# Haian-Jin/TensoIR

Hardware: AMD Instinct MI355X
Metric: primary+secondary rays/sec at 4096 rays x 512 samples (higher is better)
Workload: dtype f32 io and field; decoders split-bf16 x3 (hi/lo operands, 3 MFMA products), fp32 accumulate; indirect light (secondary-ray records): fp16 shadow taps + fp16 single-product decoder, fp32 accumulate

## Files before the change

### include/tensoir_hip.h

```cpp
#ifndef TENSOIR_HIP_H
#define TENSOIR_HIP_H

#include <stdint.h>

#ifdef __cplusplus
extern "C" {
#endif

#define TIR_VERSION 100

#define TIR_OK               0
#define TIR_ERR_ARG         -1001
#define TIR_ERR_UNSUPPORTED -1002
#define TIR_ERR_NO_DEVICE   -1003

typedef struct TirField {
    float aabb_min[3];
    float aabb_max[3];
    float inv_aabb[3];
    int32_t grid[3];
    float step_size;
    float distance_scale;
    float density_shift;
    float weight_thres;
// ... 66 lines not shown
int tir_vm_density_fwd(const TirField* f, const float* xyz, float* feat, float* sigma,
                       int64_t n, void* stream);

int tir_occupancy_query(const TirField* f, const float* xyz, uint8_t* hit, int64_t n, void* stream);

int tir_dense_alpha(const TirField* f, const float* lin_x, const float* lin_y, const float* lin_z,
                    int32_t gx, int32_t gy, int32_t gz, float length, float* alpha, void* stream);
int tir_alpha_pool(const float* alpha, int32_t gx, int32_t gy, int32_t gz, float thres, float* vol,
                   int32_t* bbox, void* stream);
int tir_filter_rays(const TirField* f, const float* rays, int64_t n, int32_t n_samples, int32_t bbox_only,
                    uint8_t* mask, void* stream);

int tir_dense_sigma_build(const TirField* f, float* vol, int32_t pitch, void* stream);
int tir_dense_sigma_fwd(const TirField* f, const float* xyz, float* feat, float* sigma, int64_t n, void* stream);

int tir_dense_app_build(const TirField* f, void* vol, int32_t pitch, void* stream);

int tir_density_grad_fwd(const TirField* f, const float* xyz, float* sigma, float* grad,
                         float* normal, int64_t n, const int32_t* n_dev, void* stream);
int tir_density_feat_grad_fwd(const TirField* f, const float* xyz, float* feat, float* grad, int64_t n, void* stream);

int tir_vm_app_fwd(const TirField* f, const float* xyz, const int32_t* light_idx,
                   const int32_t* idx_map, float* rad_feat, float* int_feat, int32_t out_stride,
                   int32_t idx_div, int64_t n, const int32_t* n_dev, void* stream);

int tir_vm_app_jitter_fwd(const TirField* f, const float* xyz, int64_t n, const int32_t* n_dev, float scale,
                          uint64_t seed, uint64_t offset, const int64_t* rng_state, float* xyz_out,
                          float* int_feat, int32_t out_stride, void* stream);

int tir_vm_app_primary_fwd(const TirField* f, const float* xyz, const int32_t* light_idx, const int32_t* idx_map,
                           float* rad_feat, float* int_feat, int32_t out_stride, int64_t n, const int32_t* n_dev,
                           float scale, uint64_t seed, uint64_t offset, const int64_t* rng_state, float* xyz_out,
                           float* int_feat_jit, void* stream);
int tir_vm_app_primary_x3_fwd(const TirField* f, const float* xyz, const int32_t* light_idx, const int32_t* idx_map,
                              float* rad_feat, float* int_feat, int32_t out_stride, int64_t n, const int32_t* n_dev,
                              float scale, uint64_t seed, uint64_t offset, const int64_t* rng_state, float* xyz_out,
                              float* int_feat_jit, void* stream);
int tir_vm_app_fwd_x3(const TirField* f, const float* xyz, const int32_t* light_idx,
                      const int32_t* idx_map, float* rad_feat, float* int_feat, int32_t out_stride,
                      int32_t idx_div, int64_t n, const int32_t* n_dev, void* stream);
int tir_vm_app_fwd_bf16x3(const TirField* f, const float* xyz, const int32_t* light_idx,
                          const int32_t* idx_map, float* rad_feat, float* int_feat, int32_t out_stride,
                          int32_t idx_div, int64_t n, const int32_t* n_dev, void* stream);
int tir_vm_app_fwd_valu(const TirField* f, const float* xyz, const int32_t* light_idx,
                        const int32_t* idx_map, float* rad_feat, float* int_feat, int32_t out_stride,
                        int32_t idx_div, int64_t n, const int32_t* n_dev, void* stream);

int tir_mlp_fwd(const TirMlp* m, const float* feat, int32_t feat_stride, const float* aux,
                const int32_t* aux_map, int32_t aux_mod, float* out, int64_t n, const int32_t* n_dev,
        void* stream);
int tir_mlp_fwd_bf16x3(const TirMlp* m, const float* feat, int32_t feat_stride, const float* aux,
                       const int32_t* aux_map, int32_t aux_mod, float* out, int64_t n, const int32_t* n_dev,
        void* stream);

int tir_pack_half(const float* const* srcs, void* const* dsts, const int64_t* counts, int32_t n_tables, void* stream);
int tir_pack_half_checked(const float* const* srcs, void* const* dsts, const int64_t* counts, int32_t n_tables, float* absmax,
                          void* stream);
int tir_vm_app_fwd_h16(const TirField* f, const TirFieldHalf* fh, const float* xyz, const int32_t* light_idx,
                       const int32_t* idx_map, float* rad_feat, int32_t out_stride, int32_t idx_div, int64_t n,
                       const int32_t* n_dev, void* stream);

int tir_indirect_fused_fwd(const TirField* f, const TirFieldHalf* fh, const TirMlp* m, const float* xyz,
                           const int32_t* light_idx, const int32_t* rec_map, int32_t idx_div, int32_t aux_mod,
                           const float* table, float* out, int64_t n, const int32_t* n_dev, void* stream);

int tir_indirect_fused_hp_fwd(const TirField* f, const TirMlp* m, const float* xyz, const int32_t* light_idx,
// ... 434 lines not shown
```

### tensoir_amd/csrc/tir_common.hpp

```cpp
#pragma once
#include <hip/hip_runtime.h>
#include <stdint.h>
#include <initializer_list>
#include <type_traits>
#include "tensoir_hip.h"

#define TIR_WAVE 64

#define TIR_CHECK_LAUNCH()                                   \
    do {                                                     \
        hipError_t e__ = hipGetLastError();                  \
        if (e__ != hipSuccess) return -(int)e__;             \
    } while (0)

static inline hipStream_t tir_stream(void* s) { return reinterpret_cast<hipStream_t>(s); }

static inline int tir_xcd_mapping(const TirField* f) { return f->tune_xcd_order == 1 ? 1 : 0; }

#include <mutex>
#include <set>
#include <utility>
static inline int tir_allow_dynamic_lds(const void* kernel, int bytes) {
    static std::mutex mu;
    static std::set<std::pair<const void*, int>> done;
// ... 65 lines not shown
    int n_acomp = 0;
    int app_dim = 0;
    bool feature_rows = true;
    int stride_max = 32;
    TirAppNeeds& fp16_tables(const TirFieldHalf* fh) { half = fh; return *this; }
    TirAppNeeds& aligned() { aligned16 = true; return *this; }
    TirAppNeeds& no_light_mean() { light_mean = false; return *this; }
    TirAppNeeds& element_index32() { index32 = true; return *this; }
    TirAppNeeds& width(int n) { n_acomp = n; return *this; }
    TirAppNeeds& app_dim_is(int d) { app_dim = d; return *this; }
    TirAppNeeds& no_feature_rows() { feature_rows = false; return *this; }
    TirAppNeeds& stride_unbounded() { stride_max = 0x7fffffff; return *this; }
};

static inline int tir_check_app_field(const TirField* f, const TirAppNeeds& need, int out_stride) {
    for (int i = 0; i < 3; ++i) {
        const void* plane = need.half ? need.half->aplane[i] : static_cast<const void*>(f->aplane[i]);
        const void* line = need.half ? need.half->aline[i] : static_cast<const void*>(f->aline[i]);
        if (f->grid[i] < 2 || !plane || !line || (need.aligned16 && !tir_aligned16({plane, line}))) return TIR_ERR_ARG;
    }
    if (!f->basis_t || !f->light_line || (need.light_mean && !f->light_mean)) return TIR_ERR_ARG;
    if (need.n_acomp && f->n_acomp != need.n_acomp) return TIR_ERR_UNSUPPORTED;
    if (need.app_dim ? f->app_dim != need.app_dim : (f->app_dim < 1 || f->app_dim > 27)) return TIR_ERR_UNSUPPORTED;
    if (need.index32 && !tir_app_index_ok(f)) return TIR_ERR_UNSUPPORTED;
    if (need.feature_rows && (out_stride < f->app_dim || out_stride > need.stride_max)) return TIR_ERR_ARG;
    return TIR_OK;
}

template <typename Go>
static inline int tir_with_rows(int64_t n, std::initializer_list<const void*> need, std::initializer_list<const void*> aligned, Go&& go) {
    if (n < 0 || (n > 0 && tir_any_null(need)) || !tir_aligned16(aligned)) return TIR_ERR_ARG;
    if (n == 0) return TIR_OK;
    return go();
}

constexpr int TIR_APP_LDS_LIMIT = 160 * 1024;

static inline unsigned tir_gather_blocks(int64_t n, int rows, int cap, int xcd_on) {
    int64_t blocks = (n + rows - 1) / rows;
    if (blocks > cap) blocks = cap;
    if (xcd_on) blocks = (blocks + 7) / 8 * 8;
    return (unsigned)blocks;
}

static inline unsigned tir_job_split(int64_t units, int total, int n_jobs) {
    int per = total / n_jobs;
    if (per < 1) per = 1;
    if (units < per) per = (int)units;
    return (unsigned)(per * n_jobs);
}

template <typename... P, typename... A>
static inline int tir_launch(void (*kernel)(P...), int lds_limit, dim3 grid, dim3 block, size_t lds, hipStream_t s, const A&... args) {
    if (lds_limit > 0)
        if (int rc = tir_allow_dynamic_lds(reinterpret_cast<const void*>(kernel), lds_limit)) return rc;
    hipLaunchKernelGGL(kernel, grid, block, lds, s, args...);
    TIR_CHECK_LAUNCH();
    return TIR_OK;
}

template <int... C4S, typename Fn>
static inline int tir_dispatch_c4(int n_acomp, Fn&& fn) {
    int rc = TIR_ERR_UNSUPPORTED;
    (void)((n_acomp == 4 * C4S && ((rc = fn(std::integral_constant<int, C4S>{})), true)) || ...);
    return rc;
}
// ... 810 lines not shown
```

### tensoir_amd/csrc/tir_field.hip

```cpp
#include "tir_common.hpp"

using namespace tir;

__global__ void k_pack_plane(const float* __restrict__ src, float* __restrict__ dst, int C, int HW) {
    int64_t i = (int64_t)blockIdx.x * blockDim.x + threadIdx.x;
    if (i >= (int64_t)C * HW) return;
    int c = (int)(i % C);
    int64_t t = i / C;
    dst[i] = src[(int64_t)c * HW + t];
}

__global__ void k_pack_occ(const float* __restrict__ vol, uint8_t* __restrict__ nbr, int W, int H, int D) {
    int64_t i = (int64_t)blockIdx.x * blockDim.x + threadIdx.x;
    const int64_t n = (int64_t)(W + 1) * (H + 1) * (D + 1);
    if (i >= n) return;
    const int x0 = (int)(i % (W + 1)) - 1, y0 = (int)((i / (W + 1)) % (H + 1)) - 1, z0 = (int)(i / ((int64_t)(W + 1) * (H + 1))) - 1;
    uint32_t m = 0;
    for (int c = 0; c < 8; ++c) {
        const int xx = x0 + (c & 1), yy = y0 + ((c >> 1) & 1), zz = z0 + (c >> 2);
        if (xx >= 0 && xx < W && yy >= 0 && yy < H && zz >= 0 && zz < D && vol[((int64_t)zz * H + yy) * W + xx] > 0.5f) m |= 1u << c;
    }
    nbr[i] = (uint8_t)m;
}

// ... 234 lines not shown

extern "C" int tir_dense_sigma_fwd(const TirField* f, const float* xyz, float* feat, float* sigma, int64_t n, void* stream) {
    int rc = check_field(f);
    if (rc) return rc;
    if (n < 0 || (n > 0 && !xyz)) return TIR_ERR_ARG;
    if (!tir_dense_sigma_ok(f)) return TIR_ERR_UNSUPPORTED;
    if (n == 0) return TIR_OK;
    hipLaunchKernelGGL(k_dense_sigma_fwd, dim3((unsigned)((n + 255) / 256)), dim3(256), 0, tir_stream(stream), *f, xyz, feat, sigma, n);
    TIR_CHECK_LAUNCH();
    return TIR_OK;
}

extern "C" int tir_alpha_pool(const float* alpha, int32_t gx, int32_t gy, int32_t gz, float thres, float* vol,
                              int32_t* bbox, void* stream) {
    if (!alpha || !vol || gx <= 0 || gy <= 0 || gz <= 0) return TIR_ERR_ARG;
    const int64_t n = (int64_t)gx * gy * gz;
    hipLaunchKernelGGL(k_alpha_pool, dim3((unsigned)((n + 255) / 256)), dim3(256), 0, tir_stream(stream), alpha, gx, gy,
                       gz, thres, vol, bbox);
    TIR_CHECK_LAUNCH();
    return TIR_OK;
}

extern "C" int tir_filter_rays(const TirField* f, const float* rays, int64_t n, int32_t n_samples, int32_t bbox_only,
                               uint8_t* mask, void* stream) {
    if (!f || n < 0 || (n > 0 && (!rays || !mask))) return TIR_ERR_ARG;
    if (!bbox_only && (!f->occ_nbr || n_samples <= 0)) return TIR_ERR_ARG;
    if (n == 0) return TIR_OK;
    hipLaunchKernelGGL(k_filter_rays, dim3((unsigned)((n + 3) / 4)), dim3(256), 0, tir_stream(stream), *f, rays, n,
                       n_samples, bbox_only, mask);
    TIR_CHECK_LAUNCH();
    return TIR_OK;
}

template <int C4>
__device__ __forceinline__ void plane_line_grad(const float* __restrict__ plane, const float* __restrict__ line,
                                                int H, int W, int R, float u, float v, float w,
                                                float& val, float& du, float& dv, float& dw) {
    Tap1 tx = make_tap(u, W), ty = make_tap(v, H), tl = make_tap(w, R);
    const float wx0 = 1.0f - tx.t, wx1 = tx.t, wy0 = 1.0f - ty.t, wy1 = ty.t;
    const float* p00 = plane + ((size_t)ty.i0 * W + tx.i0) * (C4 * 4);
    const float* p01 = plane + ((size_t)ty.i0 * W + tx.i1) * (C4 * 4);
    const float* p10 = plane + ((size_t)ty.i1 * W + tx.i0) * (C4 * 4);
    const float* p11 = plane + ((size_t)ty.i1 * W + tx.i1) * (C4 * 4);
    const float* l0 = line + (size_t)tl.i0 * (C4 * 4);
    const float* l1 = line + (size_t)tl.i1 * (C4 * 4);
    const float sx = 0.5f * (float)(W - 1), sy = 0.5f * (float)(H - 1), sl = 0.5f * (float)(R - 1);
    float a_val = 0.f, a_du = 0.f, a_dv = 0.f, a_dw = 0.f;
#pragma unroll
    for (int c = 0; c < C4 * 4; ++c) {
        float a = p00[c], b = p01[c], cc = p10[c], d = p11[c], e = l0[c], g = l1[c];
        float P = fmaf(d, wx1 * wy1, fmaf(cc, wx0 * wy1, fmaf(b, wx1 * wy0, a * (wx0 * wy0))));
        float Pu = fmaf(d - cc, wy1, (b - a) * wy0);
        float Pv = fmaf(d - b, wx1, (cc - a) * wx0);
        float L = fmaf(g, tl.t, e * (1.0f - tl.t));
        float Lw = g - e;
        a_val = fmaf(P, L, a_val);
        a_du = fmaf(Pu, L, a_du);
        a_dv = fmaf(Pv, L, a_dv);
        a_dw = fmaf(P, Lw, a_dw);
    }
    val = a_val; du = a_du * sx; dv = a_dv * sy; dw = a_dw * sl;
}

template <int C4>
__global__ void __launch_bounds__(256)
k_density_grad(TirField f, const float* __restrict__ xyz, float* __restrict__ sigma,
               float* __restrict__ grad, float* __restrict__ normal, int64_t n, const int32_t* __restrict__ n_dev) {
    int64_t i = (int64_t)blockIdx.x * blockDim.x + threadIdx.x;
    if (n_dev) n = min(n, (int64_t)max(*n_dev, 0));
    if (i >= n) return;
    const float px = xyz[3 * i], py = xyz[3 * i + 1], pz = xyz[3 * i + 2];
    float g0 = 0.f, g1 = 0.f, g2 = 0.f;
    float feat = 0.f;
#pragma unroll 1
    for (int k = 0; k < 3; ++k) {
        const float u = (k == 2) ? py : px, v = (k == 0) ? py : pz, w = (k == 0) ? pz : ((k == 1) ? py : px);
        const int m0 = (k == 2) ? 1 : 0, m1 = (k == 0) ? 1 : 2, vi = 2 - k;
        float val, du, dv, dw;
        plane_line_grad<C4>(f.dplane[k], f.dline[k], f.grid[m1], f.grid[m0], f.grid[vi], u, v, w, val, du, dv, dw);
        feat += val;
        if (k == 0) { g0 += du; g1 += dv; g2 += dw; }
        else if (k == 1) { g0 += du; g2 += dv; g1 += dw; }
        else { g1 += du; g2 += dv; g0 += dw; }
    }
    const float g[3] = {g0, g1, g2};
    float ds, sg;
    if (f.act == 1) { sg = fmaxf(feat, 0.f); ds = feat > 0.f ? 1.f : 0.f; }
    else {
        float x = feat + f.density_shift;
        sg = softplus20(x);
        ds = (x > 20.f) ? 1.f : 1.0f / (1.0f + expf(-x));
    }
    float gx = ds * g[0], gy = ds * g[1], gz = ds * g[2];
    if (sigma) sigma[i] = sg;
    if (grad) { grad[3 * i] = gx; grad[3 * i + 1] = gy; grad[3 * i + 2] = gz; }
    if (normal) {
        float nrm = fmaxf(sqrtf(gx * gx + gy * gy + gz * gz), 1e-6f);
        normal[3 * i] = -gx / nrm; normal[3 * i + 1] = -gy / nrm; normal[3 * i + 2] = -gz / nrm;
    }
}

extern "C" int tir_density_grad_fwd(const TirField* f, const float* xyz, float* sigma, float* grad,
                                    float* normal, int64_t n, const int32_t* n_dev, void* stream) {
    int rc = check_field(f);
    if (rc) return rc;
    if (n < 0 || (n > 0 && !xyz)) return TIR_ERR_ARG;
    if (n == 0) return TIR_OK;
    dim3 g((unsigned)((n + 255) / 256)), b(256);
    switch (f->n_dcomp) {
        case 16: hipLaunchKernelGGL(k_density_grad<4>, g, b, 0, tir_stream(stream), *f, xyz, sigma, grad, normal, n, n_dev); break;
        case 8:  hipLaunchKernelGGL(k_density_grad<2>, g, b, 0, tir_stream(stream), *f, xyz, sigma, grad, normal, n, n_dev); break;
        case 32: hipLaunchKernelGGL(k_density_grad<8>, g, b, 0, tir_stream(stream), *f, xyz, sigma, grad, normal, n, n_dev); break;
        default: hipLaunchKernelGGL(k_density_grad<1>, g, b, 0, tir_stream(stream), *f, xyz, sigma, grad, normal, n, n_dev); break;
    }
    TIR_CHECK_LAUNCH();
    return TIR_OK;
}

template <int C4>
__global__ void __launch_bounds__(256)
k_density_feat_grad(TirField f, const float* __restrict__ xyz, float* __restrict__ feat, float* __restrict__ grad, int64_t n) {
    int64_t i = (int64_t)blockIdx.x * blockDim.x + threadIdx.x;
    if (i >= n) return;
    const float p[3] = {xyz[3 * i], xyz[3 * i + 1], xyz[3 * i + 2]};
    float g[3] = {0.f, 0.f, 0.f}, acc = 0.f;
#pragma unroll 1
    for (int k = 0; k < 3; ++k) {
        const int m0 = (k == 2) ? 1 : 0, m1 = (k == 0) ? 1 : 2, vi = 2 - k;
        float val, du, dv, dw;
        plane_line_grad<C4>(f.dplane[k], f.dline[k], f.grid[m1], f.grid[m0], f.grid[vi], p[m0], p[m1], p[vi], val, du, dv, dw);
        acc += val;
        g[m0] += du; g[m1] += dv; g[vi] += dw;
// ... 331 lines not shown
}

template <int C4, bool HX = false>
__global__ void __launch_bounds__(256)
k_vm_app_primary(TirField f, const float* __restrict__ xyz, const int32_t* __restrict__ light_idx,
                 const int32_t* __restrict__ idx_map, float* __restrict__ rad_feat, float* __restrict__ int_feat,
                 float* __restrict__ int_feat_jit, int out_stride, int64_t n, const int32_t* __restrict__ n_dev, int xcd_on,
                 TirJitter jt, int lt_rows, int nb0) {
    if ((int)blockIdx.x < nb0) {
        TirJitter none{0.0f, 0ull, 0ull, nullptr, nullptr};
        app_mfma_body<C4, true, true, false, HX>(f, xyz, light_idx, idx_map, rad_feat, int_feat, out_stride, 0, n, n_dev, xcd_on, none,
                                                 lt_rows, (int)blockIdx.x, nb0);
    } else {
        app_mfma_body<C4, false, true, true, HX>(f, xyz, nullptr, nullptr, nullptr, int_feat_jit, out_stride, 0, n, n_dev, xcd_on, jt,
                                                 lt_rows, (int)blockIdx.x - nb0, (int)gridDim.x - nb0);
    }
}

template <int C4, bool HX = false>
__global__ void __launch_bounds__(256)
k_vm_app_primary_one(TirField f, const float* __restrict__ xyz, float* __restrict__ rad_feat, float* __restrict__ int_feat,
                     float* __restrict__ int_feat_jit, int out_stride, int64_t n, const int32_t* __restrict__ n_dev, int xcd_on,
                     TirJitter jt, int nb0) {
    if ((int)blockIdx.x < nb0) {
        TirJitter none{0.0f, 0ull, 0ull, nullptr, nullptr};
        app_mfma_body<C4, true, true, false, HX, true>(f, xyz, nullptr, nullptr, rad_feat, int_feat, out_stride, 0, n, n_dev, xcd_on, none,
                                                       1, (int)blockIdx.x, nb0);
    } else {
        app_mfma_body<C4, false, true, true, HX>(f, xyz, nullptr, nullptr, nullptr, int_feat_jit, out_stride, 0, n, n_dev, xcd_on, jt,
                                                 0, (int)blockIdx.x - nb0, (int)gridDim.x - nb0);
    }
}

typedef __bf16 app_bf16x8 __attribute__((ext_vector_type(8)));
#define TIR_XS 68

__device__ __forceinline__ void app_split8(const float4& v0, const float4& v1, app_bf16x8& hi, app_bf16x8& lo) {
    const float v[8] = {v0.x, v0.y, v0.z, v0.w, v1.x, v1.y, v1.z, v1.w};
#pragma unroll
    for (int e = 0; e < 8; ++e) {
        hi[e] = (__bf16)v[e];
        lo[e] = (__bf16)(v[e] - (float)hi[e]);
    }
}

template <int C4, bool RAD, bool INTR>
__global__ void __launch_bounds__(256)
k_vm_app_bf16(TirField f, const float* __restrict__ xyz, const int32_t* __restrict__ light_idx,
              const int32_t* __restrict__ idx_map, float* __restrict__ rad_feat, float* __restrict__ int_feat,
              int out_stride, int idx_div, int64_t n, const int32_t* __restrict__ n_dev, int xcd_on) {
    static_assert(C4 * 4 <= 64, "one VM group must fit two 32-wide k-steps");
    if (n_dev) n = min(n, (int64_t)max(*n_dev, 0));
    constexpr int CA = C4 * 4;
    constexpr int NX = (RAD ? 1 : 0) + (INTR ? 1 : 0);
    extern __shared__ __attribute__((aligned(16))) float lds_app[];
    app_bf16x8* Whi = reinterpret_cast<app_bf16x8*>(lds_app);
    app_bf16x8* Wlo = Whi + 3 * 2 * 2 * 64;
    const int wave = threadIdx.x >> 6, L = threadIdx.x & 63;
    float* X = reinterpret_cast<float*>(Wlo + 3 * 2 * 2 * 64) + wave * (NX * 16 * TIR_XS);
    for (int e = threadIdx.x; e < 3 * 2 * 2 * 64; e += 256) {
        const int row = e & 15, kg = (e >> 4) & 3, mt = (e >> 6) & 1, t = (e >> 7) & 1, k = e >> 8;
        app_bf16x8 hi, lo;
#pragma unroll
        for (int q = 0; q < 8; ++q) {
            const int ch = 32 * t + 8 * kg + q;
            const float w = (ch < CA) ? f.basis_t[(size_t)(k * CA + ch) * 32 + mt * 16 + row] : 0.0f;
// ... 320 lines not shown
static int app_fwd(const TirField* f, const float* xyz, const int32_t* li, const int32_t* map, float* rad, float* intr,
                   int32_t stride, int32_t idx_div, int64_t n, const int32_t* n_dev, void* stream, AppContraction how,
                   const TirJitter& jt = TirJitter{0.0f, 0ull, 0ull, nullptr, nullptr}) {
    if (!f) return TIR_ERR_ARG;
    if (int rc = tir_check_app_field(f, TirAppNeeds(), stride)) return rc;
    if ((!rad && !intr) || (rad && !li)) return TIR_ERR_ARG;
    return tir_with_rows(n, {xyz}, {}, [&] {
        hipStream_t s = tir_stream(stream);
        if (how == APP_BF16X3) return tir_dispatch_c4<12, 6, 4>(f->n_acomp, [&](auto c4) { return launch_app_bf16<decltype(c4)::value>(f, xyz, li, map, rad, intr, stride, idx_div, n, n_dev, s); });
        if (how == APP_HX) return tir_dispatch_c4<12, 6, 4>(f->n_acomp, [&](auto c4) { return launch_app_hx<decltype(c4)::value>(f, xyz, li, map, rad, intr, stride, idx_div, n, n_dev, s); });
        return tir_dispatch_c4<12, 6, 4, 24>(f->n_acomp, [&](auto c4) { return launch_app<decltype(c4)::value>(f, xyz, li, map, rad, intr, stride, idx_div, n, n_dev, s, how == APP_VALU, jt); });
    });
}
#undef TIR_APP_ARGS

extern "C" int tir_vm_app_fwd(const TirField* f, const float* xyz, const int32_t* light_idx,
                              const int32_t* idx_map, float* rad_feat, float* int_feat, int32_t out_stride,
                              int32_t idx_div, int64_t n, const int32_t* n_dev, void* stream) {
    return app_fwd(f, xyz, light_idx, idx_map, rad_feat, int_feat, out_stride, idx_div, n, n_dev, stream, APP_FP32);
}

extern "C" int tir_vm_app_jitter_fwd(const TirField* f, const float* xyz, int64_t n, const int32_t* n_dev, float scale,
                                     uint64_t seed, uint64_t offset, const int64_t* rng_dev, float* xyz_out,
                                     float* int_feat, int32_t out_stride, void* stream) {
    if (!xyz_out || !int_feat || scale == 0.0f) return TIR_ERR_ARG;
    TirJitter jt{scale, (unsigned long long)seed, (unsigned long long)offset, reinterpret_cast<const long long*>(rng_dev), xyz_out};
    return app_fwd(f, xyz, nullptr, nullptr, nullptr, int_feat, out_stride, 0, n, n_dev, stream, APP_FP32, jt);
}

template <bool HX>
static int app_primary_fwd(const TirField* f, const float* xyz, const int32_t* light_idx, const int32_t* idx_map, float* rad_feat,
                           float* int_feat, int32_t out_stride, int64_t n, const int32_t* n_dev, float scale, uint64_t seed,
                           uint64_t offset, const int64_t* rng_state, float* xyz_out, float* int_feat_jit, void* stream) {
    if (!f || !rad_feat || !int_feat || !xyz_out || !int_feat_jit || !light_idx || scale == 0.0f) return TIR_ERR_ARG;
    if (int rc = tir_check_app_field(f, TirAppNeeds().width(48), out_stride)) return rc;
    return tir_with_rows(n, {xyz}, {}, [&] {
        constexpr int C4 = 12, CA = 48;
        const int lt_rows = f->n_lights <= 16 ? f->n_lights : 0;
        const size_t w_floats = HX ? (2 * 3 * 2 * 2 * 64 * 16) / 4 : 3 * CA * 32;
        const size_t x_floats = HX ? (2 * 2 * 16 * TIR_XHX * 2) / 4 : 2 * CA * TIR_XLD;
        const int nb = (int)tir_gather_blocks(n, 64, 1024, 1);
        const dim3 g(2 * nb), b(256);
        const int xcd_on = tir_xcd_mapping(f);
        const TirJitter jt{scale, (unsigned long long)seed, (unsigned long long)offset, reinterpret_cast<const long long*>(rng_state), xyz_out};
        if (f->n_lights == 1) {
            const size_t lds1 = (w_floats + (size_t)2 * 3 * CA + 4 * (x_floats / 2)) * sizeof(float);
            return tir_launch(k_vm_app_primary_one<C4, HX>, TIR_APP_LDS_LIMIT, g, b, lds1, tir_stream(stream), *f, xyz, rad_feat, int_feat,
                              int_feat_jit, out_stride, n, n_dev, xcd_on, jt, nb);
        }
        const size_t lds = (w_floats + (size_t)(lt_rows + 1) * 3 * CA + 4 * x_floats) * sizeof(float);
        return tir_launch(k_vm_app_primary<C4, HX>, TIR_APP_LDS_LIMIT, g, b, lds, tir_stream(stream), *f, xyz, light_idx, idx_map, rad_feat,
                          int_feat, int_feat_jit, out_stride, n, n_dev, xcd_on, jt, lt_rows, nb);
    });
}

extern "C" int tir_vm_app_primary_fwd(const TirField* f, const float* xyz, const int32_t* light_idx, const int32_t* idx_map,
                                      float* rad_feat, float* int_feat, int32_t out_stride, int64_t n, const int32_t* n_dev,
                                      float scale, uint64_t seed, uint64_t offset, const int64_t* rng_state, float* xyz_out,
                                      float* int_feat_jit, void* stream) {
    return app_primary_fwd<false>(f, xyz, light_idx, idx_map, rad_feat, int_feat, out_stride, n, n_dev, scale, seed, offset, rng_state,
                                  xyz_out, int_feat_jit, stream);
}

extern "C" int tir_vm_app_primary_x3_fwd(const TirField* f, const float* xyz, const int32_t* light_idx, const int32_t* idx_map,
                                         float* rad_feat, float* int_feat, int32_t out_stride, int64_t n, const int32_t* n_dev,
                                         float scale, uint64_t seed, uint64_t offset, const int64_t* rng_state, float* xyz_out,
                                         float* int_feat_jit, void* stream) {
    return app_primary_fwd<true>(f, xyz, light_idx, idx_map, rad_feat, int_feat, out_stride, n, n_dev, scale, seed, offset, rng_state,
                                 xyz_out, int_feat_jit, stream);
}

extern "C" int tir_vm_app_fwd_x3(const TirField* f, const float* xyz, const int32_t* light_idx,
                                 const int32_t* idx_map, float* rad_feat, float* int_feat, int32_t out_stride,
                                 int32_t idx_div, int64_t n, const int32_t* n_dev, void* stream) {
    return app_fwd(f, xyz, light_idx, idx_map, rad_feat, int_feat, out_stride, idx_div, n, n_dev, stream, APP_HX);
}

extern "C" int tir_vm_app_fwd_valu(const TirField* f, const float* xyz, const int32_t* light_idx,
                                   const int32_t* idx_map, float* rad_feat, float* int_feat, int32_t out_stride,
                                   int32_t idx_div, int64_t n, const int32_t* n_dev, void* stream) {
    return app_fwd(f, xyz, light_idx, idx_map, rad_feat, int_feat, out_stride, idx_div, n, n_dev, stream, APP_VALU);
}

extern "C" int tir_vm_app_fwd_bf16x3(const TirField* f, const float* xyz, const int32_t* light_idx,
                                     const int32_t* idx_map, float* rad_feat, float* int_feat, int32_t out_stride,
// ... 74 lines not shown
```

### tensoir_amd/field_model.py

```python
from __future__ import annotations

import functools
import math
import time

import numpy as np
import torch
import torch.nn as nn
import torch.nn.functional as F

from . import capacity, indirect, ops, regularisers
from ._lib import TensoirHipError, TirField

MAT_MODE = [[0, 1], [0, 2], [1, 2]]
VEC_MODE = [2, 1, 0]


def raw2alpha(sigma, dist):
    alpha = 1.0 - torch.exp(-sigma * dist)
    T = torch.cumprod(torch.cat([torch.ones(alpha.shape[0], 1).to(alpha.device), 1.0 - alpha + 1e-10], -1), -1)
    weights = alpha * T[:, :-1]
    return alpha, weights, T[:, -1:]


# ... 849 lines not shown
        f = self.packed_field()
        lidx = ops.to_device(light_idx.reshape(-1), dev, torch.int32).contiguous()
        jitter = ops.to_device(torch.rand(B, 1), dev) if is_train else None
        from . import training
        if training.wants_grad(self):
            bg = bool(white_bg or (is_train and torch.rand((1,)) < 0.5))
            for attempt in range(2):
                try:
                    maps = training.PrimaryRenderFn.apply(self, rays, lidx, S, bg, bool(is_relight), jitter,
                                                          _brdf_jitter_dense, bool(_defer_check),
                                                          *training.field_param_list(self))
                    break
                except training._CapacityOverflow:
                    if attempt:
                        raise
            out = self.unpack_maps(maps, is_relight, want_mask=_want_mask)
            return (out, maps) if _return_maps else out
        rc = capacity.PassCapacity(self.__dict__.setdefault("_app_cap_hints", {}), (B, S), 1.25, ceiling=B * S, max_entries=64,
                                   capture=self.__dict__.get("_capture"), check_key=("primary", B, S))
        cap = rc.hinted() if (not is_train and _brdf_jitter_dense is None) else None
        words = viewdirs = None
        if cap is None:
            weight, acc, depth, _tend, cnt = ops.march_primary(f, rays, jitter, S, self.march_t_stop)
            offsets = ops.exclusive_scan(cnt)
            A, n_dev = int(offsets[-1].item()), None
        else:
            words = self._step_words(dev)
            weight, acc, depth, cnt, offsets, total_dev, viewdirs = ops.march_primary_fused(f, rays, S, self.march_t_stop,
                                                                                            cap, words)
            self.__dict__["_rec_counter_armed"] = words[1:3]
            A, n_dev = cap, offsets[B:]
            rc.watch(total_dev, cap)
        rec_ray, rec_k, rec_w, rec_xyz = ops.compact_primary(f, rays, jitter, weight, offsets, A)
        rgb = brdf = brdf_j = pred = derived = None
        rng_state = None
        if A > 0:
            if viewdirs is None:
                viewdirs = rays[:, 3:6].contiguous()
            merged = bool(is_relight) and _brdf_jitter_dense is None and f.n_acomp == 48 and ops.APP_IMPL == "mfma"
            if merged:
                rng_state = self._jitter_rng(dev)
                rad, intr, xyz_j, intr_j = ops.vm_app_primary(f, rec_xyz, lidx, rec_ray, 0.01, rng_state, n_dev)
            else:
                rad, intr = ops.vm_app(f, rec_xyz, lidx, rec_ray, True, bool(is_relight), None, 0, n_dev)
            jobs = [(self.renderModule.packed(), rad, viewdirs, rec_ray)]
            if is_relight:
                pb = self.renderModule_brdf.packed()
                jobs.append((pb, intr, rec_xyz, None))
                if merged:
                    pass
                elif _brdf_jitter_dense is not None:
                    noise = _brdf_jitter_dense.to(dev, torch.float32)[rec_ray.long(), rec_k.long()]
                    xyz_j = torch.add(rec_xyz, noise, alpha=0.01)
                    intr_j = ops.vm_app(f, xyz_j, None, None, False, True, None, 0, n_dev)[1]
                else:
                    rng_state = self._jitter_rng(dev)
                    xyz_j, intr_j = ops.vm_app_jitter(f, rec_xyz, 0.01, 0, 0, rng_state, n_dev)
                jobs.append((pb, intr_j, xyz_j, None))
                if self.normals_kind in ("purely_predicted", "derived_plus_predicted"):
                    jobs.append((self.renderModule_normal.packed(), intr, rec_xyz, None))
            if ops.MLP_IMPL == "bf16x3":
                outs = ops.mlp_multi(jobs, n_dev)
            else:
                outs = [ops.mlp(m, ft, ax, mp, None, 0, n_dev) for m, ft, ax, mp in jobs]
            rgb = outs[0]
            if is_relight:
                brdf, brdf_j = outs[1], outs[2]
                if self.normals_kind == "purely_derived":
                    pred = ops.density_grad(f, rec_xyz, n_dev=n_dev)[2]
                elif self.normals_kind == "gt_normals":
                    pred = None
                elif self.normals_kind == "residue_prediction":
                    derived = ops.density_grad(f, rec_xyz, n_dev=n_dev)[2]
                    pred = self.renderModule_normal.rows(rec_xyz, derived, intr, n_dev)
                else:
                    pred = outs[3]
                    if self.normals_kind == "derived_plus_predicted":
                        derived = ops.density_grad(f, rec_xyz, n_dev=n_dev)[2]
        bg = bool(white_bg or (is_train and torch.rand((1,)) < 0.5))
        smooth = None
        if words is not None:
            maps, smooth = ops.composite_primary_fused(rays, offsets, rec_w, rgb, brdf, brdf_j, pred, derived, acc, depth,
                                                       bg, is_relight, self.fixed_fresnel, words, rng_state, 1)
        else:
            maps = ops.composite_primary(rays, offsets, rec_w, rgb, brdf, brdf_j, pred, derived, acc, depth,
                                         bg, is_relight, self.fixed_fresnel)
            if rng_state is not None:
                rng_state[1] += 1
        if self.normals_kind not in NORMAL_LOSS_KINDS and is_relight:
            maps[:, 16] = 0.0

        if rc.capture is None:
            finish = rc.settle if words is not None else functools.partial(rc.settle, A)
            if _defer_check:
                self.__dict__["_pending_primary"] = finish
            elif not finish():
                return self.forward(rays_chunk, light_idx, white_bg, is_train, ndc_ray, is_relight, N_samples,
                                    _brdf_jitter_dense, _return_maps, False, _want_mask)
        out = self.unpack_maps(maps, is_relight, want_mask=_want_mask, smooth=smooth)
        return (out, maps) if _return_maps else out

    def _step_words(self, dev):
        w = self.__dict__.get("_words")
        if w is None or w.device != torch.device(dev):
            w = self.__dict__["_words"] = torch.zeros((8,), dtype=torch.int32, device=dev)
            self.__dict__["_pair_counter"] = w[0:1]
        return w

    def _jitter_rng(self, dev):
        seed = int(torch.cuda.initial_seed())
        st = self.__dict__.get("_jit_rng")
# ... 29 lines not shown
```

### tensoir_amd/ops.py

```python
from __future__ import annotations

import ctypes as C
import math
import os

import numpy as np
import torch

from . import _lib
from ._lib import TirEnvSG, TirField, TirFieldHalf, TirMlp, check, lib

_K = _lib.CONST
MAP_STRIDE = _K["TIR_MAP_STRIDE"]

STATS = None
TIMING = None

TUNE = {
    "dense_app": 0 if os.environ.get("TENSOIR_DENSE_APP", "1") == "0" else 1,
    "dense_app_max_mb": max(0, int(os.environ.get("TENSOIR_DENSE_APP_MAX_MB", "4096") or 0)),
    "lds_lines": 2 if os.environ.get("TENSOIR_LDS_LINES", "1") == "0" else 0,
    "xcd_order": 1 if os.environ.get("TIR_XCD", "0") == "1" else 0,
    "dense_sigma": 0 if os.environ.get("TENSOIR_DENSE_SIGMA", "1") == "0" else 1,
    "dense_sigma_max_mb": max(0, int(os.environ.get("TENSOIR_DENSE_SIGMA_MAX_MB", "1024") or 0)),
# ... 567 lines not shown
          C.c_void_p(words.data_ptr() + 4), 2, C.c_void_p(words.data_ptr() + 12), _ptr(off), int(cap), _ptr(total), _stream())
    return weight, acc, depth, cnt, off, total, vd


def composite_primary_fused(rays, offsets, rec_w, rgb, brdf, brdf_jit, pred_n, der_n, acc, depth, white_bg, is_relight,
                            fixed_fresnel, words, rng_state=None, rng_step=0):
    rays = f32(rays, "rays", 6)
    B = rays.shape[0]
    out = torch.empty((B, MAP_STRIDE), dtype=torch.float32, device=rays.device)
    smooth = torch.zeros((2,), dtype=torch.float32, device=rays.device) if B == 0 else \
        torch.empty((2,), dtype=torch.float32, device=rays.device)
    _call("tir_composite_primary_fused", _ptr(rays), _ptr(offsets), _ptr(rec_w), _ptr(rgb), _ptr(brdf), _ptr(brdf_jit),
          _ptr(pred_n), _ptr(der_n), _ptr(acc), _ptr(depth), B, int(bool(white_bg)), int(bool(is_relight)),
          float(fixed_fresnel), _ptr(out), C.c_void_p(words.data_ptr() + 16), _ptr(smooth), _ptr(rng_state), int(rng_step),
          _stream())
    return out, smooth


def vm_app_jitter(field: TirField, xyz, scale, seed, offset, rng_state=None, n_dev=None):
    xyz = f32(xyz, "xyz", 3).view(-1, 3)
    n = xyz.shape[0]
    xyz_j = torch.empty_like(xyz)
    intr = torch.empty((n, FEAT_STRIDE), dtype=torch.float32, device=xyz.device)
    _call("tir_vm_app_jitter_fwd", C.byref(field), _ptr(xyz), n, _ptr(n_dev), float(scale), int(seed) & (2 ** 64 - 1),
          int(offset) & (2 ** 64 - 1), _ptr(rng_state), _ptr(xyz_j), _ptr(intr), FEAT_STRIDE, _stream())
    return xyz_j, intr


APP_CONTRACTION = os.environ.get("TENSOIR_APP_CONTRACTION", "fp32")
if APP_CONTRACTION not in ("x3", "fp32"):
    raise ValueError(f"TENSOIR_APP_CONTRACTION={APP_CONTRACTION!r}: expected x3 or fp32")


def app_contraction():
    return APP_CONTRACTION if MLP_IMPL == "bf16x3" else "fp32"


def vm_app_primary(field: TirField, xyz, light_idx, idx_map, scale, rng_state, n_dev=None, exact=False):
    xyz = f32(xyz, "xyz", 3).view(-1, 3)
    n = xyz.shape[0]
    dev = xyz.device
    rad = torch.empty((n, FEAT_STRIDE), dtype=torch.float32, device=dev)
    intr = torch.empty((n, FEAT_STRIDE), dtype=torch.float32, device=dev)
    intr_j = torch.empty((n, FEAT_STRIDE), dtype=torch.float32, device=dev)
    xyz_j = torch.empty_like(xyz)
    _call("tir_vm_app_primary_fwd" if (exact or app_contraction() == "fp32") else "tir_vm_app_primary_x3_fwd", C.byref(field), _ptr(xyz),
          _ptr(i32(light_idx, "light_idx").view(-1)),
          _ptr(None if idx_map is None else i32(idx_map, "idx_map").view(-1)), _ptr(rad), _ptr(intr), FEAT_STRIDE, n, _ptr(n_dev),
          float(scale), 0, 0, _ptr(rng_state), _ptr(xyz_j), _ptr(intr_j), _stream())
    return rad, intr, xyz_j, intr_j


def exclusive_scan(counts):
    counts = i32(counts, "counts").view(-1)
    n = counts.numel()
    off = torch.empty((n + 1,), dtype=torch.int32, device=counts.device)
    _call("tir_exclusive_scan", _ptr(counts), _ptr(off), n, _stream())
    return off


def exclusive_scan_capped(counts, cap):
    counts = i32(counts, "counts").view(-1)
    n = counts.numel()
    off = torch.empty((n + 1,), dtype=torch.int32, device=counts.device)
    total = torch.empty((1,), dtype=torch.int32, device=counts.device)
    _call("tir_exclusive_scan_capped", _ptr(counts), _ptr(off), n, int(cap), _ptr(total), _stream())
    return off, total


def compact_primary(field: TirField, rays, ray_jitter, weight, offsets, total, out=None):
    rays = f32(rays, "rays", 6)
    B, S = weight.shape
    dev = rays.device
    if ray_jitter is not None:
        ray_jitter = f32(ray_jitter, "ray_jitter").view(-1)
    if out is not None:
        rec_ray, rec_k, rec_w, rec_xyz = i32(out[0], "rec_ray"), i32(out[1], "rec_k"), f32(out[2], "rec_w"), f32(out[3], "rec_xyz", 3)
        if min(rec_ray.numel(), rec_k.numel(), rec_w.numel(), rec_xyz.shape[0]) < total:
            raise ValueError("compact_primary: out buffers hold fewer than `total` records")
    else:
        rec_ray = torch.empty((total,), dtype=torch.int32, device=dev)
        rec_k = torch.empty((total,), dtype=torch.int32, device=dev)
        rec_w = torch.empty((total,), dtype=torch.float32, device=dev)
# ... 1674 lines not shown
```

Baseline: 6.100 million.

## Fuse density-gradient normal computation into merged primary appearance kernel launch

Adds extra blocks to the merged primary appearance kernel that compute derived normals from the density gradient, so one launch covers work that previously needed a separate density_grad call. The request is passed through a thread-local pointer set by a new entry point. This removes a kernel launch and lets the gradient work overlap with the MFMA appearance blocks. In exchange it raises register and LDS pressure (launch bounds 256,3), adds sched barriers, and changes the summation order of the normal to explicit round-to-nearest ops.

After: 6.029 million. -1.2%, worse.

```diff
diff --git a/include/tensoir_hip.h b/include/tensoir_hip.h
--- a/include/tensoir_hip.h
+++ b/include/tensoir_hip.h
@@ -122,6 +122,7 @@
                            float* rad_feat, float* int_feat, int32_t out_stride, int64_t n, const int32_t* n_dev,
                            float scale, uint64_t seed, uint64_t offset, const int64_t* rng_state, float* xyz_out,
                            float* int_feat_jit, void* stream);
+int tir_vm_app_primary_normal(float* normal);
 int tir_vm_app_primary_x3_fwd(const TirField* f, const float* xyz, const int32_t* light_idx, const int32_t* idx_map,
                               float* rad_feat, float* int_feat, int32_t out_stride, int64_t n, const int32_t* n_dev,
                               float scale, uint64_t seed, uint64_t offset, const int64_t* rng_state, float* xyz_out,
diff --git a/tensoir_amd/csrc/tir_common.hpp b/tensoir_amd/csrc/tir_common.hpp
--- a/tensoir_amd/csrc/tir_common.hpp
+++ b/tensoir_amd/csrc/tir_common.hpp
@@ -121,6 +121,11 @@
     if (n < 0 || (n > 0 && tir_any_null(need)) || !tir_aligned16(aligned)) return TIR_ERR_ARG;
     if (n == 0) return TIR_OK;
     return go();
+}
+
+inline float*& tir_primary_normal_request() {
+    static thread_local float* normal = nullptr;
+    return normal;
 }
 
 constexpr int TIR_APP_LDS_LIMIT = 160 * 1024;
diff --git a/tensoir_amd/csrc/tir_field.hip b/tensoir_amd/csrc/tir_field.hip
--- a/tensoir_amd/csrc/tir_field.hip
+++ b/tensoir_amd/csrc/tir_field.hip
@@ -290,7 +290,7 @@
     return TIR_OK;
 }
 
-template <int C4>
+template <int C4, bool HALVES = false>
 __device__ __forceinline__ void plane_line_grad(const float* __restrict__ plane, const float* __restrict__ line,
                                                 int H, int W, int R, float u, float v, float w,
                                                 float& val, float& du, float& dv, float& dw) {
@@ -306,6 +306,7 @@
     float a_val = 0.f, a_du = 0.f, a_dv = 0.f, a_dw = 0.f;
 #pragma unroll
     for (int c = 0; c < C4 * 4; ++c) {
+        if (HALVES && c == C4 * 2) __builtin_amdgcn_sched_barrier(0);
         float a = p00[c], b = p01[c], cc = p10[c], d = p11[c], e = l0[c], g = l1[c];
         float P = fmaf(d, wx1 * wy1, fmaf(cc, wx0 * wy1, fmaf(b, wx1 * wy0, a * (wx0 * wy0))));
         float Pu = fmaf(d - cc, wy1, (b - a) * wy0);
@@ -320,13 +321,10 @@
     val = a_val; du = a_du * sx; dv = a_dv * sy; dw = a_dw * sl;
 }
 
-template <int C4>
-__global__ void __launch_bounds__(256)
-k_density_grad(TirField f, const float* __restrict__ xyz, float* __restrict__ sigma,
-               float* __restrict__ grad, float* __restrict__ normal, int64_t n, const int32_t* __restrict__ n_dev) {
-    int64_t i = (int64_t)blockIdx.x * blockDim.x + threadIdx.x;
-    if (n_dev) n = min(n, (int64_t)max(*n_dev, 0));
-    if (i >= n) return;
+template <int C4, bool SLICE = false>
+__device__ __forceinline__ void
+density_grad_row(const TirField& f, const float* __restrict__ xyz, float* __restrict__ sigma, float* __restrict__ grad,
+                 float* __restrict__ normal, const int64_t i) {
     const float px = xyz[3 * i], py = xyz[3 * i + 1], pz = xyz[3 * i + 2];
     float g0 = 0.f, g1 = 0.f, g2 = 0.f;
     float feat = 0.f;
@@ -335,11 +333,17 @@
         const float u = (k == 2) ? py : px, v = (k == 0) ? py : pz, w = (k == 0) ? pz : ((k == 1) ? py : px);
         const int m0 = (k == 2) ? 1 : 0, m1 = (k == 0) ? 1 : 2, vi = 2 - k;
         float val, du, dv, dw;
-        plane_line_grad<C4>(f.dplane[k], f.dline[k], f.grid[m1], f.grid[m0], f.grid[vi], u, v, w, val, du, dv, dw);
+        plane_line_grad<C4, (SLICE && C4 >= 4)>(f.dplane[k], f.dline[k], f.grid[m1], f.grid[m0], f.grid[vi], u, v, w, val, du, dv, dw);
         feat += val;
-        if (k == 0) { g0 += du; g1 += dv; g2 += dw; }
-        else if (k == 1) { g0 += du; g2 += dv; g1 += dw; }
-        else { g1 += du; g2 += dv; g0 += dw; }
+        if constexpr (SLICE) {
+            if (k == 0) { g0 = add_rn(g0, du); g1 = add_rn(g1, dv); g2 = add_rn(g2, dw); }
+            else if (k == 1) { g0 = add_rn(g0, du); g2 = add_rn(g2, dv); g1 = add_rn(g1, dw); }
+            else { g1 = add_rn(g1, du); g2 = add_rn(g2, dv); g0 = add_rn(g0, dw); }
+        } else {
+            if (k == 0) { g0 += du; g1 += dv; g2 += dw; }
+            else if (k == 1) { g0 += du; g2 += dv; g1 += dw; }
+            else { g1 += du; g2 += dv; g0 += dw; }
+        }
     }
     const float g[3] = {g0, g1, g2};
     float ds, sg;
@@ -353,9 +357,19 @@
     if (sigma) sigma[i] = sg;
     if (grad) { grad[3 * i] = gx; grad[3 * i + 1] = gy; grad[3 * i + 2] = gz; }
     if (normal) {
-        float nrm = fmaxf(sqrtf(gx * gx + gy * gy + gz * gz), 1e-6f);
+        float nrm = fmaxf(sqrtf(add_rn(mul_rn(gz, gz), fmaf(gy, gy, mul_rn(gx, gx)))), 1e-6f);
         normal[3 * i] = -gx / nrm; normal[3 * i + 1] = -gy / nrm; normal[3 * i + 2] = -gz / nrm;
     }
+}
+
+template <int C4>
+__global__ void __launch_bounds__(256)
+k_density_grad(TirField f, const float* __restrict__ xyz, float* __restrict__ sigma,
+               float* __restrict__ grad, float* __restrict__ normal, int64_t n, const int32_t* __restrict__ n_dev) {
+    int64_t i = (int64_t)blockIdx.x * blockDim.x + threadIdx.x;
+    if (n_dev) n = min(n, (int64_t)max(*n_dev, 0));
+    if (i >= n) return;
+    density_grad_row<C4>(f, xyz, sigma, grad, normal, i);
 }
 
 extern "C" int tir_density_grad_fwd(const TirField* f, const float* xyz, float* sigma, float* grad,
@@ -753,6 +767,53 @@
     }
 }
 
+template <int D4>
+__device__ __forceinline__ void
+density_grad_slice(const TirField& f, const float* __restrict__ xyz, float* __restrict__ normal, int64_t n,
+                   const int32_t* __restrict__ n_dev, int xcd_on, const int bid, const int nblk) {
+    if (n_dev) n = min(n, (int64_t)max(*n_dev, 0));
+    const XcdRange xr = xcd_range_at((n + 255) / 256, 1, xcd_on != 0, bid, nblk);
+    for (int64_t tile = xr.first; tile < xr.end; tile += xr.stride) {
+        const int64_t i = tile * 256 + threadIdx.x;
+        if (i < n) density_grad_row<D4, true>(f, xyz, nullptr, nullptr, normal, i);
+    }
+}
+
+template <int C4, int D4>
+__global__ void __launch_bounds__(256, 3)
+k_vm_app_primary_grad(TirField f, const float* __restrict__ xyz, const int32_t* __restrict__ light_idx,
+                      const int32_t* __restrict__ idx_map, float* __restrict__ rad_feat, float* __restrict__ int_feat,
+                      float* __restrict__ int_feat_jit, float* __restrict__ normal, int out_stride, int64_t n,
+                      const int32_t* __restrict__ n_dev, int xcd_on, TirJitter jt, int lt_rows, int nb0) {
+    if ((int)blockIdx.x < nb0) {
+        TirJitter none{0.0f, 0ull, 0ull, nullptr, nullptr};
+        app_mfma_body<C4, true, true, false, false>(f, xyz, light_idx, idx_map, rad_feat, int_feat, out_stride, 0, n, n_dev, xcd_on, none,
+                                                 lt_rows, (int)blockIdx.x, nb0);
+    } else if ((int)blockIdx.x < 2 * nb0) {
+        app_mfma_body<C4, false, true, true, false>(f, xyz, nullptr, nullptr, nullptr, int_feat_jit, out_stride, 0, n, n_dev, xcd_on, jt,
+                                                 lt_rows, (int)blockIdx.x - nb0, nb0);
+    } else {
+        density_grad_slice<D4>(f, xyz, normal, n, n_dev, xcd_on, (int)blockIdx.x - 2 * nb0, (int)gridDim.x - 2 * nb0);
+    }
+}
+
+template <int C4, int D4>
+__global__ void __launch_bounds__(256, 3)
+k_vm_app_primary_one_grad(TirField f, const float* __restrict__ xyz, float* __restrict__ rad_feat, float* __restrict__ int_feat,
+                          float* __restrict__ int_feat_jit, float* __restrict__ normal, int out_stride, int64_t n,
+                          const int32_t* __restrict__ n_dev, int xcd_on, TirJitter jt, int nb0) {
+    if ((int)blockIdx.x < nb0) {
+        TirJitter none{0.0f, 0ull, 0ull, nullptr, nullptr};
+        app_mfma_body<C4, true, true, false, false, true>(f, xyz, nullptr, nullptr, rad_feat, int_feat, out_stride, 0, n, n_dev, xcd_on, none,
+                                                       1, (int)blockIdx.x, nb0);
+    } else if ((int)blockIdx.x < 2 * nb0) {
+        app_mfma_body<C4, false, true, true, false>(f, xyz, nullptr, nullptr, nullptr, int_feat_jit, out_stride, 0, n, n_dev, xcd_on, jt,
+                                                 0, (int)blockIdx.x - nb0, nb0);
+    } else {
+        density_grad_slice<D4>(f, xyz, normal, n, n_dev, xcd_on, (int)blockIdx.x - 2 * nb0, (int)gridDim.x - 2 * nb0);
+    }
+}
+
 typedef __bf16 app_bf16x8 __attribute__((ext_vector_type(8)));
 #define TIR_XS 68
 
@@ -1139,6 +1200,7 @@
 static int app_primary_fwd(const TirField* f, const float* xyz, const int32_t* light_idx, const int32_t* idx_map, float* rad_feat,
                            float* int_feat, int32_t out_stride, int64_t n, const int32_t* n_dev, float scale, uint64_t seed,
                            uint64_t offset, const int64_t* rng_state, float* xyz_out, float* int_feat_jit, void* stream) {
+    float* const normal = std::exchange(tir_primary_normal_request(), nullptr);
     if (!f || !rad_feat || !int_feat || !xyz_out || !int_feat_jit || !light_idx || scale == 0.0f) return TIR_ERR_ARG;
     if (int rc = tir_check_app_field(f, TirAppNeeds().width(48), out_stride)) return rc;
     return tir_with_rows(n, {xyz}, {}, [&] {
@@ -1150,14 +1212,33 @@
         const dim3 g(2 * nb), b(256);
         const int xcd_on = tir_xcd_mapping(f);
         const TirJitter jt{scale, (unsigned long long)seed, (unsigned long long)offset, reinterpret_cast<const long long*>(rng_state), xyz_out};
+        const size_t lds1 = (w_floats + (size_t)2 * 3 * CA + 4 * (x_floats / 2)) * sizeof(float);
+        const size_t lds = (w_floats + (size_t)(lt_rows + 1) * 3 * CA + 4 * x_floats) * sizeof(float);
+        if (normal) {
+            if (int rc = check_field(f)) return rc;
+            if constexpr (!HX) {
+                const dim3 g3(2 * nb + tir_gather_blocks(n, 256, 1024, 1));
+                const int rc = tir_dispatch_c4<4, 2>(f->n_dcomp, [&](auto d4) {
+                    constexpr int D4 = decltype(d4)::value;
+                    if (f->n_lights == 1)
+                        return tir_launch(k_vm_app_primary_one_grad<C4, D4>, TIR_APP_LDS_LIMIT, g3, b, lds1, tir_stream(stream), *f, xyz,
+                                          rad_feat, int_feat, int_feat_jit, normal, out_stride, n, n_dev, xcd_on, jt, nb);
+                    return tir_launch(k_vm_app_primary_grad<C4, D4>, TIR_APP_LDS_LIMIT, g3, b, lds, tir_stream(stream), *f, xyz, light_idx,
+                                      idx_map, rad_feat, int_feat, int_feat_jit, normal, out_stride, n, n_dev, xcd_on, jt, lt_rows, nb);
+                });
+                if (rc != TIR_ERR_UNSUPPORTED) return rc;
+            }
+        }
+        int rc;
         if (f->n_lights == 1) {
-            const size_t lds1 = (w_floats + (size_t)2 * 3 * CA + 4 * (x_floats / 2)) * sizeof(float);
-            return tir_launch(k_vm_app_primary_one<C4, HX>, TIR_APP_LDS_LIMIT, g, b, lds1, tir_stream(stream), *f, xyz, rad_feat, int_feat,
-                              int_feat_jit, out_stride, n, n_dev, xcd_on, jt, nb);
-        }
-        const size_t lds = (w_floats + (size_t)(lt_rows + 1) * 3 * CA + 4 * x_floats) * sizeof(float);
-        return tir_launch(k_vm_app_primary<C4, HX>, TIR_APP_LDS_LIMIT, g, b, lds, tir_stream(stream), *f, xyz, light_idx, idx_map, rad_feat,
-                          int_feat, int_feat_jit, out_stride, n, n_dev, xcd_on, jt, lt_rows, nb);
+            rc = tir_launch(k_vm_app_primary_one<C4, HX>, TIR_APP_LDS_LIMIT, g, b, lds1, tir_stream(stream), *f, xyz, rad_feat, int_feat,
+                            int_feat_jit, out_stride, n, n_dev, xcd_on, jt, nb);
+        } else {
+            rc = tir_launch(k_vm_app_primary<C4, HX>, TIR_APP_LDS_LIMIT, g, b, lds, tir_stream(stream), *f, xyz, light_idx, idx_map, rad_feat,
+                            int_feat, int_feat_jit, out_stride, n, n_dev, xcd_on, jt, lt_rows, nb);
+        }
+        if (rc || !normal) return rc;
+        return tir_density_grad_fwd(f, xyz, nullptr, nullptr, normal, n, n_dev, stream);
     });
 }
 
diff --git a/tensoir_amd/csrc/tir_primary.hip b/tensoir_amd/csrc/tir_primary.hip
--- /dev/null
+++ b/tensoir_amd/csrc/tir_primary.hip
@@ -0,0 +1,6 @@
+#include "tir_common.hpp"
+
+extern "C" int tir_vm_app_primary_normal(float* normal) {
+    tir_primary_normal_request() = normal;
+    return TIR_OK;
+}
diff --git a/tensoir_amd/field_model.py b/tensoir_amd/field_model.py
--- a/tensoir_amd/field_model.py
+++ b/tensoir_amd/field_model.py
@@ -905,7 +905,7 @@
             A, n_dev = cap, offsets[B:]
             rc.watch(total_dev, cap)
         rec_ray, rec_k, rec_w, rec_xyz = ops.compact_primary(f, rays, jitter, weight, offsets, A)
-        rgb = brdf = brdf_j = pred = derived = None
+        rgb = brdf = brdf_j = pred = derived = sliced_normal = None
         rng_state = None
         if A > 0:
             if viewdirs is None:
@@ -913,7 +913,12 @@
             merged = bool(is_relight) and _brdf_jitter_dense is None and f.n_acomp == 48 and ops.APP_IMPL == "mfma"
             if merged:
                 rng_state = self._jitter_rng(dev)
-                rad, intr, xyz_j, intr_j = ops.vm_app_primary(f, rec_xyz, lidx, rec_ray, 0.01, rng_state, n_dev)
+                sliced = ops.PRIMARY_NORMAL_SLICE and self.normals_kind in ("purely_derived", "derived_plus_predicted",
+                                                                             "residue_prediction")
+                rad, intr, xyz_j, intr_j, *rest = ops.vm_app_primary(f, rec_xyz, lidx, rec_ray, 0.01, rng_state, n_dev,
+                                                                     want_normal=sliced)
+                if sliced:
+                    sliced_normal = rest[0]
             else:
                 rad, intr = ops.vm_app(f, rec_xyz, lidx, rec_ray, True, bool(is_relight), None, 0, n_dev)
             jobs = [(self.renderModule.packed(), rad, viewdirs, rec_ray)]
@@ -939,17 +944,18 @@
             rgb = outs[0]
             if is_relight:
                 brdf, brdf_j = outs[1], outs[2]
+                derive = lambda: sliced_normal if sliced_normal is not None else ops.density_grad(f, rec_xyz, n_dev=n_dev)[2]
                 if self.normals_kind == "purely_derived":
-                    pred = ops.density_grad(f, rec_xyz, n_dev=n_dev)[2]
+                    pred = derive()
                 elif self.normals_kind == "gt_normals":
                     pred = None
                 elif self.normals_kind == "residue_prediction":
-                    derived = ops.density_grad(f, rec_xyz, n_dev=n_dev)[2]
+                    derived = derive()
                     pred = self.renderModule_normal.rows(rec_xyz, derived, intr, n_dev)
                 else:
                     pred = outs[3]
                     if self.normals_kind == "derived_plus_predicted":
-                        derived = ops.density_grad(f, rec_xyz, n_dev=n_dev)[2]
+                        derived = derive()
         bg = bool(white_bg or (is_train and torch.rand((1,)) < 0.5))
         smooth = None
         if words is not None:
diff --git a/tensoir_amd/ops.py b/tensoir_amd/ops.py
--- a/tensoir_amd/ops.py
+++ b/tensoir_amd/ops.py
@@ -623,11 +623,14 @@
     raise ValueError(f"TENSOIR_APP_CONTRACTION={APP_CONTRACTION!r}: expected x3 or fp32")
 
 
+PRIMARY_NORMAL_SLICE = True
+
+
 def app_contraction():
     return APP_CONTRACTION if MLP_IMPL == "bf16x3" else "fp32"
 
 
-def vm_app_primary(field: TirField, xyz, light_idx, idx_map, scale, rng_state, n_dev=None, exact=False):
+def vm_app_primary(field: TirField, xyz, light_idx, idx_map, scale, rng_state, n_dev=None, exact=False, want_normal=False):
     xyz = f32(xyz, "xyz", 3).view(-1, 3)
     n = xyz.shape[0]
     dev = xyz.device
@@ -635,11 +638,15 @@
     intr = torch.empty((n, FEAT_STRIDE), dtype=torch.float32, device=dev)
     intr_j = torch.empty((n, FEAT_STRIDE), dtype=torch.float32, device=dev)
     xyz_j = torch.empty_like(xyz)
+    normal = None
+    if want_normal:
+        normal = torch.empty_like(xyz)
+        _call("tir_vm_app_primary_normal", _ptr(normal))
     _call("tir_vm_app_primary_fwd" if (exact or app_contraction() == "fp32") else "tir_vm_app_primary_x3_fwd", C.byref(field), _ptr(xyz),
           _ptr(i32(light_idx, "light_idx").view(-1)),
           _ptr(None if idx_map is None else i32(idx_map, "idx_map").view(-1)), _ptr(rad), _ptr(intr), FEAT_STRIDE, n, _ptr(n_dev),
           float(scale), 0, 0, _ptr(rng_state), _ptr(xyz_j), _ptr(intr_j), _stream())
-    return rad, intr, xyz_j, intr_j
+    return (rad, intr, xyz_j, intr_j, normal) if want_normal else (rad, intr, xyz_j, intr_j)
 
 
 def exclusive_scan(counts):
```
